# lichunshang/vision-enhanced-lidar-odometry

Hardware: AMD Instinct MI355X
Metric: scan-pairs/sec + achieved HBM GB/s, 120k-pt HDL-64E frame-to-frame ICP (higher is better)
Workload: dtype f32 association / f64 residuals+solve

## Files before the change

vision-enhanced-lidar-odometry_amd/csrc/velo_kernels.h:

```cpp
#pragma once
#include <hip/hip_runtime.h>
#include <stdint.h>

#include "velo_device_math.h"

#ifndef VELO_DEF_LOAD
#define VELO_DEF_LOAD 0
#endif
#ifndef VELO_DEF_ASSOC
#define VELO_DEF_ASSOC 0
#endif
#ifndef VELO_DEF_LMA
#define VELO_DEF_LMA 0
#endif
#ifndef VELO_DEF_LMB
#define VELO_DEF_LMB 0
#endif

namespace velo {

constexpr int kWave = 64;
constexpr int kNumAcc = 28;
constexpr int kEvalThreads = 256;
constexpr int kMaxEvalBlocks = 512;
// ... 490 lines not shown
    for (int off = 1; off < 64; off <<= 1) {
#pragma unroll
        for (int k = 0; k < kSub; k++) { const int t = __shfl_up(inc[k], off); if (lane >= off) inc[k] += t; }
    }
    if (lane == 63) {
#pragma unroll
        for (int k = 0; k < kSub; k++) s_wsum[k][wid] = inc[k];
    }
    __syncthreads();
    int ex[kSub], run = 0;
#pragma unroll
    for (int k = 0; k < kSub; k++) {
        int before = 0, all = 0;
#pragma unroll
        for (int w = 0; w < kWaves; w++) { const int sw = s_wsum[k][w]; if (w < wid) before += sw; all += sw; }
        ex[k] = run + before + inc[k] - ((v[k].x + v[k].y) + (v[k].z + v[k].w));
        run += all;
    }
    const int total = run;
    if (threadIdx.x == 0) {
        s_prefix = 0;
        __hip_atomic_store(&status[tile], (tile == 0 ? kLbPrefix : kLbAgg) | (unsigned long long)(unsigned)total, __ATOMIC_RELAXED, __HIP_MEMORY_SCOPE_AGENT);
    }
    if (tile > 0 && threadIdx.x < 64) {
        int acc = 0;
        for (int idx = tile - 1;; idx -= 64) {
            const int j = idx - lane;
            unsigned long long w = kLbPrefix;
            if (j >= 0) { do { w = __hip_atomic_load(&status[j], __ATOMIC_RELAXED, __HIP_MEMORY_SCOPE_AGENT); } while ((w & kLbFlags) == 0ull); }
            const unsigned long long pm = __ballot((w & kLbFlags) == kLbPrefix);
            const int first = (int)__ffsll((long long)pm) - 1;
            int val = (pm == 0ull || lane <= first) ? (int)(unsigned)(w & 0xffffffffull) : 0;
#pragma unroll
            for (int off = 32; off > 0; off >>= 1) val += __shfl_xor(val, off);
            acc += val;
            if (pm != 0ull) break;
        }
        if (lane == 0) {
            s_prefix = acc;
            __hip_atomic_store(&status[tile], kLbPrefix | (unsigned long long)(unsigned)(acc + total), __ATOMIC_RELAXED, __HIP_MEMORY_SCOPE_AGENT);
        }
    }
    __syncthreads();
    const int pre = s_prefix;
#pragma unroll
    for (int k = 0; k < kSub; k++) {
        const int i = tbase + k * (kScanThreads * 4) + threadIdx.x * 4;
        int4 q;
        q.x = pre + ex[k]; q.y = q.x + v[k].x; q.z = q.y + v[k].y; q.w = q.z + v[k].z;
        if (i + 3 < n) *reinterpret_cast<int4*>(data + i) = q;
        else { if (i < n) data[i] = q.x; if (i + 1 < n) data[i + 1] = q.y; if (i + 2 < n) data[i + 2] = q.z; }
        if (i <= n - 1 && n - 1 < i + 4) *grand_total = q.w + v[k].w;
    }
}
template <int kLbItems>
__global__ void __launch_bounds__(kScanThreads)
scan_lookback_kernel(int* __restrict__ data, int n, unsigned long long* __restrict__ status, int* __restrict__ ticket, int* __restrict__ grand_total) {
    scan_lookback_body<kLbItems>(data, n, status, ticket, grand_total);
}
__global__ void scan_tiles_kernel(int* __restrict__ data, int n, int* __restrict__ tile_sums)
#if VELO_DEF_LOAD
{
    const int base = blockIdx.x * kScanTile + threadIdx.x * kScanItems;
    int v[kScanItems], s = 0;
#pragma unroll
    for (int k = 0; k < kScanItems; k++) { v[k] = (base + k < n) ? data[base + k] : 0; s += v[k]; }
    int total;
    int ex = block_exclusive_scan(s, &total);
#pragma unroll
    for (int k = 0; k < kScanItems; k++) { if (base + k < n) data[base + k] = ex; ex += v[k]; }
    if (threadIdx.x == 0) tile_sums[blockIdx.x] = total;
}
#else
;
#endif
__global__ void scan_sums_kernel(int* __restrict__ tile_sums, int n_tiles, int* __restrict__ grand_total)
#if VELO_DEF_LOAD
{
    __shared__ int carry_s;
    if (threadIdx.x == 0) carry_s = 0;
    __syncthreads();
    for (int start = 0; start < n_tiles; start += kScanThreads) {
        const int i = start + threadIdx.x;
        const int v = (i < n_tiles) ? tile_sums[i] : 0;
        int total;
        const int ex = block_exclusive_scan(v, &total);
        const int carry = carry_s;
        if (i < n_tiles) tile_sums[i] = ex + carry;
        __syncthreads();
        if (threadIdx.x == 0) carry_s = carry + total;
        __syncthreads();
    }
    if (threadIdx.x == 0) *grand_total = carry_s;
}
#else
;
#endif
__global__ void scan_add_kernel(int* __restrict__ data, int n, const int* __restrict__ tile_sums, const int* __restrict__ grand_total,
                                int* __restrict__ cursor)
#if VELO_DEF_LOAD
{
    const int i = blockIdx.x * blockDim.x + threadIdx.x;
    if (i < n) { const int v = data[i] + tile_sums[i / kScanTile]; data[i] = v; cursor[i] = v; }
    else if (i == n) data[n] = *grand_total;
}
#else
;
#endif
__device__ __forceinline__ void grid_scatter_body(const float4* __restrict__ pts, const int* __restrict__ cell_of, const int* __restrict__ ring_of, int n,
                                                  int* __restrict__ cursor, const int* __restrict__ n_finite, int first_point,
                                                  float4* __restrict__ sorted, int* __restrict__ sring, const int bx) {
    const int i = bx * 256 + threadIdx.x;
    if (i < kGridPad) {
        const int j = *n_finite + i;
        sorted[j] = make_float4(__builtin_inff(), __builtin_inff(), __builtin_inff(), __int_as_float(0x7fffffff));
        sring[j] = 0x7fffffff;
    }
    const int c = i < n ? cell_of[i] : -1;
    bool head; int first, len;
    const int lane = threadIdx.x & 63;
    run_of_lane(c, lane, &head, &first, &len);
    int slot = head ? atomicAdd(&cursor[c], len) : 0;
    slot = __shfl(slot, first) + (lane - first);
    if (c < 0) return;
    const float4 p = pts[i];
    sorted[slot] = make_float4(p.x, p.y, p.z, __int_as_float(i + first_point));
    sring[slot] = ring_of[i];
}
__global__ void __launch_bounds__(256)
grid_scatter_kernel(const float4* __restrict__ pts, const int* __restrict__ cell_of, const int* __restrict__ ring_of, int n,
                    int* __restrict__ cursor, const int* __restrict__ n_finite, int first_point, float4* __restrict__ sorted, int* __restrict__ sring)
#if VELO_DEF_LOAD
{
    grid_scatter_body(pts, cell_of, ring_of, n, cursor, n_finite, first_point, sorted, sring, (int)blockIdx.x);
}
#else
;
#endif

constexpr int kAdvRings = 64, kAdvJobs = 4;
struct AdvJob {
    const float4* tgt; int* tgt_off_dev; int* ring_of; float4* pad; unsigned long long* lb_status; int* cell_of; int* table;
    float4* sorted; int* sring; int* scan_total; int* lb_ticket; int* clear; int n_clear;
    GridDesc g;
    int n_t, n_rings_t, first_ring, first_point, lb_words, nb_t, nc, n_tiles, nb_sc;
    const char* raw; long long stride; float4* src; int* src_off_dev; int* q_src; float4* qpts; unsigned* keys; unsigned* keys_next;
    unsigned* h_keys;
    float4* seed_fill;
    int n_s, n_rings_s, nb_pack, nb_q, skip, nq, patch, patch_rings, patch_len;
    int off_t[kAdvRings + 1], off_s[kAdvRings + 1];
};
struct AdvBatch { AdvJob job[kAdvJobs]; };

__global__ void __launch_bounds__(256)
advance_clear_kernel(AdvBatch B)
#if VELO_DEF_LOAD
{
    const AdvJob& J = B.job[blockIdx.y];
    int4* p = reinterpret_cast<int4*>(J.clear);
    const int n4 = J.n_clear >> 2;
    for (int i = blockIdx.x * 256 + threadIdx.x; i < n4; i += gridDim.x * 256) p[i] = make_int4(0, 0, 0, 0);
}
#else
;
#endif
__global__ void __launch_bounds__(256)
advance_ingest_kernel(AdvBatch B)
#if VELO_DEF_LOAD
{
    const AdvJob& J = B.job[blockIdx.y];
    __shared__ int s_off[kAdvRings + 2], s_qoff[kAdvRings + 2];
    __shared__ float red[4][6];
    const int tid = threadIdx.x, lane = tid & 63;
    int bx = blockIdx.x;
    if (bx < J.nb_t) {
        const int R = J.n_rings_t, n = J.n_t;
        if (tid <= R) s_off[tid] = J.off_t[tid];
        for (int j = bx * 256 + tid; j < J.lb_words; j += J.nb_t * 256) J.lb_status[j] = 0ull;
        __syncthreads();
        if (bx == 0 && tid <= R) J.tgt_off_dev[tid] = s_off[tid];
#pragma unroll
        for (int u = 0; u < kIngestPerThread; u++) {
            const int i = (bx * kIngestPerThread + u) * 256 + tid;
            int c = -1;
            if (i < n) {
                const float4 p = J.tgt[i];
                int lo = 0, hi = R;
                while (hi - lo > 1) { const int mid = (lo + hi) >> 1; if (s_off[mid] <= i) lo = mid; else hi = mid; }
                J.ring_of[i] = lo + J.first_ring;
                const int base = s_off[lo], end = s_off[lo + 1];
                J.pad[i + 2 * lo + 1] = p;
                if (i == base) J.pad[end + 2 * lo + 1] = p;
                if (i == end - 1) J.pad[base + 2 * lo] = p;
                if (isfinite(p.x) && isfinite(p.y) && isfinite(p.z)) c = cell_of_point(J.g, p);
                J.cell_of[i] = c;
            }
            bool head; int first, len;
            run_of_lane(c, lane, &head, &first, &len);
            if (head) atomicAdd(&J.table[c + 1], len);
        }
        return;
    }
    bx -= J.nb_t;
    if (bx >= J.nb_pack) return;
    const int R = J.n_rings_s;
    if (tid <= R) s_off[tid] = J.off_s[tid];
    if (tid < 64) {
        int cnt = tid < R ? (J.off_s[tid + 1] - J.off_s[tid] + J.skip - 1) / J.skip : 0;
#pragma unroll
        for (int o = 1; o < 64; o <<= 1) { const int t = __shfl_up(cnt, o); if (lane >= o) cnt += t; }
        if (tid == 0) s_qoff[0] = 0;
        if (tid < R) s_qoff[tid + 1] = cnt;
    }
    __syncthreads();
    if (bx == 0) {
        if (tid <= R) { J.src_off_dev[tid] = s_off[tid]; J.src_off_dev[R + 1 + tid] = s_qoff[tid]; }
        if (tid < 6) J.keys_next[tid] = tid < 3 ? 0xffffffffu : 0u;
    }
    if (bx >= J.nb_pack) return;
    __shared__ float s_raw[256 * 3];
    const int i = bx * 256 + tid;
    const bool have = i < J.n_s;
    const bool aligned = (reinterpret_cast<unsigned long long>(J.raw) & 15ull) == 0ull;
    float4 v = make_float4(0.f, 0.f, 0.f, 0.f);
    if (J.stride == 12 && aligned) {
        const char* base = J.raw + (long long)bx * 3072;
        const int nbytes = min(3072, (J.n_s - bx * 256) * 12);
        if (tid < 192) {
            if (tid * 16 + 16 <= nbytes) *reinterpret_cast<uint4*>(&s_raw[tid * 4]) = *reinterpret_cast<const uint4*>(base + tid * 16);
            else for (int f = 0; f < 4; f++) if (tid * 16 + 4 * f + 4 <= nbytes) s_raw[tid * 4 + f] = *reinterpret_cast<const float*>(base + tid * 16 + 4 * f);
        }
        __syncthreads();
        if (have) v = make_float4(s_raw[3 * tid], s_raw[3 * tid + 1], s_raw[3 * tid + 2], 0.0f);
    } else if (have) {
        const char* q = J.raw + (long long)i * J.stride;
        if (J.stride == 16 && aligned) { const float4 w = *reinterpret_cast<const float4*>(q); v = make_float4(w.x, w.y, w.z, 0.0f); }
        else { const float* p = reinterpret_cast<const float*>(q); v = make_float4(p[0], p[1], p[2], 0.0f); }
    }
    float mn[3] = {3.0e38f, 3.0e38f, 3.0e38f}, mx[3] = {-3.0e38f, -3.0e38f, -3.0e38f};
    if (have) {
        J.src[i] = v;
        if (isfinite(v.x) && isfinite(v.y) && isfinite(v.z)) { mn[0] = mx[0] = v.x; mn[1] = mx[1] = v.y; mn[2] = mx[2] = v.z; }
        if (J.nq > 0) {
            int lo = 0, hi = R;
            while (hi - lo > 1) { const int mid = (lo + hi) >> 1; if (s_off[mid] <= i) lo = mid; else hi = mid; }
            const int j = i - s_off[lo];
            if (j % J.skip == 0) {
                const int k = j / J.skip;
                const int pos = J.patch ? patch_position(s_qoff, R, lo, k, J.patch_rings, J.patch_len) : s_qoff[lo] + k;
                J.q_src[pos] = i;
                if (J.qpts) J.qpts[pos] = v;
                if (J.seed_fill) {
                    const float4 none = make_float4(__int_as_float(-1), __int_as_float(-1), __int_as_float(-1), __int_as_float(-1));
                    J.seed_fill[pos] = none; J.seed_fill[J.nq + pos] = none;
                }
            }
        }
    }
#pragma unroll
    for (int k = 0; k < 3; k++) {
#pragma unroll
        for (int o = 32; o > 0; o >>= 1) { mn[k] = fminf(mn[k], __shfl_xor(mn[k], o)); mx[k] = fmaxf(mx[k], __shfl_xor(mx[k], o)); }
    }
    const int wid = tid >> 6;
    if (lane == 0) { for (int k = 0; k < 3; k++) { red[wid][k] = mn[k]; red[wid][3 + k] = mx[k]; } }
    __syncthreads();
    if (tid < 6) {
        const int k = tid;
        float vv = red[0][k];
        for (int w = 1; w < 4; w++) vv = (k < 3) ? fminf(vv, red[w][k]) : fmaxf(vv, red[w][k]);
        const unsigned key = f2key(vv), cur = J.keys[k];
        if (k < 3) { if (vv < 3.0e38f && key < cur) atomicMin(&J.keys[k], key); } else { if (vv > -3.0e38f && key > cur) atomicMax(&J.keys[k], key); }
    }
}
#else
;
#endif
template <int kLbItems>
__global__ void __launch_bounds__(kScanThreads)
advance_scan_kernel(AdvBatch B) {
    const AdvJob& J = B.job[blockIdx.y];
    if ((int)blockIdx.x >= J.n_tiles) return;
    scan_lookback_body<kLbItems>(J.table + 1, J.nc, J.lb_status, J.lb_ticket, J.scan_total);
}
__global__ void __launch_bounds__(256)
advance_scatter_kernel(AdvBatch B)
#if VELO_DEF_LOAD
{
    const AdvJob& J = B.job[blockIdx.y];
    if ((int)blockIdx.x >= J.nb_sc) return;
    if (blockIdx.x == 0 && threadIdx.x < 6 && J.h_keys) J.h_keys[threadIdx.x] = J.keys[threadIdx.x];
    grid_scatter_body(J.tgt, J.cell_of, J.ring_of, J.n_t, J.table + 1, J.scan_total, J.first_point, J.sorted, J.sring, (int)blockIdx.x);
}
#else
;
#endif

struct PartialRec;
struct AssocOut {
    float4* __restrict__ p;
    float4* __restrict__ n;
    float4* __restrict__ v0;
    int4* __restrict__ aux0;
    float4* __restrict__ aux1;
    int* __restrict__ n_valid;
    int* __restrict__ n_valid_next;
    unsigned long long* __restrict__ dbg;
    unsigned long long* __restrict__ wg_times;
    int first_ring, first_point;
    struct PartialRec* __restrict__ partial;
    float4* __restrict__ prev_a;
    float4* __restrict__ prev_b;
    int2* __restrict__ prev_r;
    int* __restrict__ ask_count;
    int* __restrict__ ask_count_next;
    int* __restrict__ ask_list;
    unsigned long long* __restrict__ ask_keys;
    int2* __restrict__ ask_rings;
    int ask_map;
};

struct PartialRec {
    unsigned long long key1, key2;
    int ring1, ring2;
    int idx1, idx_k, idx2, pad;
    float v0[3], v2[3], v1[3];
    float pad2;
};

__device__ __forceinline__ float dist2_f(float qx, float qy, float qz, float sx, float sy, float sz) {
    const float dx = qx - sx, dy = qy - sy, dz = qz - sz;
    float r = dx * dx;
    r = r + dy * dy;
    r = r + dz * dz;
    return r;
}

__device__ __forceinline__ void transform_query(const PoseScalars& P, const float4& p, float* qx, float* qy, float* qz) {
    const double x = p.x, y = p.y, z = p.z;
    double r0, r1, r2;
    if (!P.small) {
        const double c0 = P.u[1] * z - P.u[2] * y, c1 = P.u[2] * x - P.u[0] * z, c2 = P.u[0] * y - P.u[1] * x;
        const double tmp = (P.u[0] * x + P.u[1] * y + P.u[2] * z) * P.omc;
        r0 = x * P.c + c0 * P.s + P.u[0] * tmp;
        r1 = y * P.c + c1 * P.s + P.u[1] * tmp;
        r2 = z * P.c + c2 * P.s + P.u[2] * tmp;
    } else {
        r0 = x + (P.w[1] * z - P.w[2] * y);
        r1 = y + (P.w[2] * x - P.w[0] * z);
        r2 = z + (P.w[0] * y - P.w[1] * x);
    }
    *qx = (float)(r0 + P.t[0]);
    *qy = (float)(r1 + P.t[1]);
    *qz = (float)(r2 + P.t[2]);
}

__device__ __forceinline__ int plane_from_points(const float v0[3], const float v1[3], const float v2[3], double norm_cond, float n[3]) {
    const float ax = v1[0] - v0[0], ay = v1[1] - v0[1], az = v1[2] - v0[2];
    const float bx = v2[0] - v0[0], by = v2[1] - v0[1], bz = v2[2] - v0[2];
    const float cx = ay * bz - az * by, cy = az * bx - ax * bz, cz = ax * by - ay * bx;
    const float nn = sqrtf(cx * cx + cy * cy + cz * cz);
    if ((double)nn < norm_cond) return 0;
    n[0] = cx / nn; n[1] = cy / nn; n[2] = cz / nn;
    return 1;
}

__device__ __forceinline__ void write_correspondence(int qi, const float4& psrc, int valid, const float n[3], const float v0[3],
                                                     int ring_i, int idx_i, int ring_j, int idx_j, int idx_k, float di, float dj,
                                                     const AssocOut& out, bool want_aux) {
    out.p[qi] = make_float4(psrc.x, psrc.y, psrc.z, __int_as_float(valid));
    out.n[qi] = valid ? make_float4(n[0], n[1], n[2], 0.f) : make_float4(0.f, 0.f, 0.f, 0.f);
    out.v0[qi] = valid ? make_float4(v0[0], v0[1], v0[2], 0.f) : make_float4(0.f, 0.f, 0.f, 0.f);
    if (want_aux) {
        out.aux0[qi] = make_int4(ring_i, idx_i, ring_j, idx_j);
        out.aux1[qi] = make_float4(__int_as_float(idx_k), di, dj, 0.f);
    }
    const unsigned long long m = __ballot(valid);
    const unsigned long long act = __ballot(1);
    if ((int)(threadIdx.x & 63) == (int)__ffsll((long long)act) - 1 && m) atomicAdd(out.n_valid, (int)__popcll(m));
}

__device__ __forceinline__ void finish_correspondence(
    int qi, const float4& psrc, float qx, float qy, float qz, unsigned long long b1, unsigned long long b2, unsigned long long key_inf,
    const float4* __restrict__ tgt, const int* __restrict__ tgt_off, const int* __restrict__ ring_of, double norm_cond,
    const AssocOut& out, bool want_aux) {
    int ring_i = -1, idx_i = 0, ring_j = -1, idx_j = 0, idx_k = 0;
    float di = 1e18f, dj = 1e18f;
    float v0[3] = {0.f, 0.f, 0.f}, v1[3] = {0.f, 0.f, 0.f}, v2[3] = {0.f, 0.f, 0.f};
    if (b1 < key_inf) {
        const int gi = (int)(unsigned)(b1 & 0xffffffffull) - out.first_point;
        ring_i = ring_of[gi];
        const int base = tgt_off[ring_i - out.first_ring];
        const int n = tgt_off[ring_i - out.first_ring + 1] - base;
        idx_i = gi - base;
        di = __uint_as_float((unsigned)(b1 >> 32));
        const int k1 = (idx_i + 1) % n, k2 = (idx_i - 1 + n) % n;
        const float4 a1 = tgt[base + k1], a2 = tgt[base + k2];
        const float d1 = dist2_f(a1.x, a1.y, a1.z, qx, qy, qz);
        const float d2 = dist2_f(a2.x, a2.y, a2.z, qx, qy, qz);
        idx_k = (d1 < d2) ? k1 : k2;
        const float4 p0 = tgt[base + idx_i];
        const float4 p2 = (idx_k == k1) ? a1 : a2;
        v0[0] = p0.x; v0[1] = p0.y; v0[2] = p0.z; v2[0] = p2.x; v2[1] = p2.y; v2[2] = p2.z;
    }
    if (b2 < key_inf) {
        const int gj = (int)(unsigned)(b2 & 0xffffffffull) - out.first_point;
        ring_j = ring_of[gj];
        idx_j = gj - tgt_off[ring_j - out.first_ring];
        dj = __uint_as_float((unsigned)(b2 >> 32));
        const float4 p1 = tgt[gj];
        v1[0] = p1.x; v1[1] = p1.y; v1[2] = p1.z;
    }
    if (out.partial) {
        PartialRec r;
        r.key1 = b1; r.key2 = b2; r.ring1 = ring_i; r.ring2 = ring_j; r.idx1 = idx_i; r.idx_k = idx_k; r.idx2 = idx_j; r.pad = 0;
        for (int k = 0; k < 3; k++) { r.v0[k] = v0[k]; r.v2[k] = v2[k]; r.v1[k] = v1[k]; }
        r.pad2 = 0.f;
        out.partial[qi] = r;
        return;
    }
    int valid = 0;
    float n[3] = {0.f, 0.f, 0.f};
    if (ring_i >= 0 && ring_j >= 0) valid = plane_from_points(v0, v1, v2, norm_cond, n);
    write_correspondence(qi, psrc, valid, n, v0, ring_i, idx_i, ring_j, idx_j, idx_k, di, dj, out, want_aux);
}

__device__ __forceinline__ void finish_correspondence_pad(
    int qi, const float4* __restrict__ qpts, float qx, float qy, float qz, unsigned long long b1, unsigned long long b2, int ring_i_in, int ring_j_in,
    unsigned long long key_inf, const float4* __restrict__ pad, const int* __restrict__ tgt_off, double norm_cond,
    const AssocOut& out, bool want_aux) {
    const bool has1 = b1 < key_inf, has2 = b2 < key_inf;
    const int gi = has1 ? (int)(unsigned)(b1 & 0xffffffffull) - out.first_point : 0;
    const int gj = has2 ? (int)(unsigned)(b2 & 0xffffffffull) - out.first_point : 0;
    const int li = has1 ? ring_i_in - out.first_ring : 0, lj = has2 ? ring_j_in - out.first_ring : 0;
    const int pi = gi + 2 * li + 1, pj = gj + 2 * lj + 1;
    const float4 psrc = qpts[qi];
    float4 p0 = make_float4(0.f, 0.f, 0.f, 0.f), p1 = p0, a1 = p0, a2 = p0;
    if (has1) { p0 = pad[pi]; a1 = pad[pi + 1]; a2 = pad[pi - 1]; }
    if (has2) p1 = pad[pj];
    int ring_i = -1, idx_i = 0, ring_j = -1, idx_j = 0, idx_k = 0;
    float di = 1e18f, dj = 1e18f;
    float v0[3] = {0.f, 0.f, 0.f}, v1[3] = {0.f, 0.f, 0.f}, v2[3] = {0.f, 0.f, 0.f};
    bool next_closer = false;
    if (has1) {
        ring_i = ring_i_in;
        di = __uint_as_float((unsigned)(b1 >> 32));
        const float d1 = dist2_f(a1.x, a1.y, a1.z, qx, qy, qz);
        const float d2 = dist2_f(a2.x, a2.y, a2.z, qx, qy, qz);
        next_closer = d1 < d2;
// ... 2781 lines not shown
    for (int i = 0; i < 6; i++) { sc[i] = S->scale[i]; gs[i] = S->g[i] * sc[i]; }
    const double scr = S->scale[r];
#pragma unroll
    for (int c = 0; c < 6; c++) {
        const double h = S->H[r <= c ? tri(r, c) : tri(c, r)];
        hrow[c] = h * scr * sc[c];
    }
    const int ei = lane < 36 ? lane / 6 : 5, ej = lane < 36 ? lane % 6 : 5;
    const double hs_e = S->H[ei <= ej ? tri(ei, ej) : tri(ej, ei)] * S->scale[ei] * S->scale[ej];
    int iter = S->iter, invalid = S->invalid, reuse = S->reuse_diag;
    double radius = S->radius, decrease = S->decrease;
    double diag_r = S->diag[r];
    for (;;) {
        if (iter + 1 > Q.max_num_iterations) { if (lane == 0) { S->done = 1; S->termination = 1; } break; }
        if (radius < Q.min_radius) { if (lane == 0) { S->done = 1; S->termination = 0; } break; }
        iter++;
        if (!reuse) {
            double hdd = hrow[0];
#pragma unroll
            for (int c = 1; c < 6; c++) hdd = (r == c) ? hrow[c] : hdd;
            diag_r = fmin(fmax(hdd, Q.min_diag), Q.max_diag);
        }
        const double inv_radius = 1.0 / radius;
        const double dterm = diag_r * inv_radius;
        double L[6], inv[6];
        bool ok = true;
#pragma unroll
        for (int j = 0; j < 6; j++) {
            double sj = (r == j) ? hrow[j] + dterm : hrow[j];
#pragma unroll
            for (int k = 0; k < j; k++) sj -= L[k] * lane_get(L[k], j);
            const double d = lane_get(sj, j);
            if (!(d > 0.0) || !isfinite(d)) { ok = false; break; }
            const double ljj = sqrt(d);
            inv[j] = 1.0 / ljj;
            L[j] = (r == j) ? ljj : sj * inv[j];
        }
        double y[6];
        if (ok) {
            double acc = gs[0];
#pragma unroll
            for (int c = 1; c < 6; c++) acc = (r == c) ? gs[c] : acc;
            double z[6];
#pragma unroll
            for (int k = 0; k < 6; k++) {
                z[k] = lane_get(acc, k) * inv[k];
                acc -= L[k] * z[k];
            }
#pragma unroll
            for (int i = 5; i >= 0; i--) {
                double sv = z[i];
#pragma unroll
                for (int k = i + 1; k < 6; k++) sv -= lane_get(L[i], k) * y[k];
                y[i] = sv * inv[i];
            }
#pragma unroll
            for (int i = 0; i < 6; i++) ok = ok && isfinite(y[i]);
        }
        reuse = 1;
        double mc = 0.0, step[6];
        if (ok) {
            double gd = 0.0, dHd = 0.0;
#pragma unroll
            for (int i = 0; i < 6; i++) step[i] = -y[i];
            double si = step[0], sj = step[0];
#pragma unroll
            for (int c = 1; c < 6; c++) { si = (ei == c) ? step[c] : si; sj = (ej == c) ? step[c] : sj; }
            const double prod = si * hs_e * sj;
#pragma unroll
            for (int i = 0; i < 6; i++) gd += gs[i] * step[i];
#pragma unroll
            for (int l = 0; l < 36; l++) dHd += lane_get(prod, l);
            mc = -(gd + 0.5 * dHd);
            if (!(mc > 0.0)) ok = false;
        }
        if (!ok) {
            if (++invalid >= Q.max_invalid) { if (lane == 0) { S->done = 1; S->termination = 2; } break; }
            radius = radius / decrease; decrease *= 2.0; reuse = 1;
            continue;
        }
        invalid = 0;
        if (lane == 0) {
            double dn = 0.0;
#pragma unroll
            for (int i = 0; i < 6; i++) { const double d = step[i] * sc[i]; S->xc[i] = S->x[i] + d; dn += d * d; }
            S->step_norm = sqrt(dn);
            S->model_change = mc;
            S->phase = PHASE_CAND;
        }
        break;
    }
    if (lane < 6) S->diag[lane] = diag_r;
    if (lane == 0) { S->iter = iter; S->invalid = invalid; S->reuse_diag = reuse; S->radius = radius; S->decrease = decrease; }
}
__device__ __forceinline__ void lm_transition_wave(const LMParams& Q, LMState* sL, const double* E, int lane) {
    int need = 0;
    if (lane == 0) {
        LMState L = *sL;
        bool ns = false;
        lm_transition_local(Q, &L, E, &ns);
        *sL = L;
        need = ns ? 1 : 0;
    }
    __builtin_amdgcn_fence(__ATOMIC_RELEASE, "wavefront");
    __builtin_amdgcn_wave_barrier();
    __builtin_amdgcn_fence(__ATOMIC_ACQUIRE, "wavefront");
    need = __builtin_amdgcn_readfirstlane(need);
    if (need) lm_compute_step_wave(Q, sL, lane);
    __builtin_amdgcn_fence(__ATOMIC_RELEASE, "wavefront");
    __builtin_amdgcn_wave_barrier();
    __builtin_amdgcn_fence(__ATOMIC_ACQUIRE, "wavefront");
}

__global__ void __launch_bounds__(256)
lm_step_kernel(LMParams Q, LMState* S, LMEvalPoint* pt, const double* __restrict__ partials, int n_blocks, unsigned long long* trace, int trace_eval,
               PoseRecord* __restrict__ pose_out, SolveLog* __restrict__ log)
#if VELO_DEF_LMA
{
    lm_transition(Q, S, pt, partials, n_blocks, trace, trace_eval, nullptr, pose_out, log);
}
#else
;
#endif
__global__ void __launch_bounds__(256)
lm_step_peer_kernel(LMParams Q, LMState* S, LMEvalPoint* pt, const double* __restrict__ partials, int n_blocks, PeerComm C,
                    PoseRecord* __restrict__ pose_out, SolveLog* __restrict__ log)
#if VELO_DEF_LMA
{
    lm_transition(Q, S, pt, partials, n_blocks, nullptr, 0, &C, pose_out, log);
}
#else
;
#endif
__global__ void lm_begin_batch_kernel(const LMBatchItem* __restrict__ items)
#if VELO_DEF_LMA
{
    const LMBatchItem& it = items[blockIdx.x];
    lm_begin_body(it.S, const_cast<LMEvalPoint*>(it.A.pt), it.xd, it.n_valid);
    if (threadIdx.x == 0 && it.pose_out) it.pose_out->ready = 0;
}
#else
;
#endif
__global__ void __launch_bounds__(256)
lm_step_batch_kernel(LMParams Q, const LMBatchItem* __restrict__ items)
#if VELO_DEF_LMA
{
    const LMBatchItem& it = items[blockIdx.x];
    lm_transition(Q, it.S, const_cast<LMEvalPoint*>(it.A.pt), it.A.partials, it.n_rows, nullptr, 0, nullptr, it.pose_out, it.log);
}
#else
;
#endif
template <bool M_LDS, int PRE, int CHUNK, bool VIS = false>
__device__ __forceinline__ void eval_step_batch_body(const LMParams& Q, const LMBatchItem& it, int* __restrict__ tickets, const int first) {
    const int bx = blockIdx.x, nbx = it.nb_icp, nb_all = VIS ? it.nb_icp + it.nb_vis : it.nb_icp;
    if (bx >= nb_all) return;
#ifdef VELO_LM_SETPRIO
    __builtin_amdgcn_s_setprio(VELO_LM_SETPRIO);
#endif
    const EvalArgs& A = it.A;
    const RowPrefetchT<PRE> f = prefetch_rows<PRE>(A, (VIS && bx >= nbx) ? 0 : bx, nbx);
    __shared__ LMEvalPoint s_pt;
    __shared__ LMState sL;
    __shared__ double s_scratch[CHUNK * kNumAcc];
    __shared__ int s_last;
    static_assert(CHUNK * kNumAcc >= kScratchDoubles / 2, "the sweep's reduction needs 64 columns x 28");
    if (first) {
        if (threadIdx.x < 4) {
            double x[6];
#pragma unroll
            for (int k = 0; k < 6; k++) x[k] = it.xd ? it.xd[k] : it.S->x[k];
            eval_point_column(x, 0, threadIdx.x, &s_pt);
        }
        __syncthreads();
    } else
    if (!eval_point_load(A, &s_pt)) return;
    double acc[kNumAcc];
    if (VIS && bx >= nbx) {
        if (M_LDS) visual_sweep_one(A, s_pt, bx - nbx, it.nb_vis, acc);
        else visual_sweep_acc(A, s_pt, bx - nbx, it.nb_vis, acc);
        block_reduce_store<true>(acc, A.partials + (size_t)(A.vis_row0 + bx - nbx) * kNumAcc, s_scratch);
    } else {
        sweep_rows<M_LDS, PRE>(A, f, s_pt, bx, nbx, acc);
        block_reduce_store<true>(acc, A.partials + (size_t)bx * kNumAcc, s_scratch);
    }
    asm volatile("s_waitcnt vmcnt(0)" ::: "memory");
    __syncthreads();
    if (threadIdx.x == 0) s_last = __hip_atomic_fetch_add(tickets + blockIdx.y, 1, __ATOMIC_RELAXED, __HIP_MEMORY_SCOPE_AGENT) == nb_all - 1 ? 1 : 0;
    __syncthreads();
    if (!s_last) return;
    if (threadIdx.x == 0) __hip_atomic_store(tickets + blockIdx.y, 0, __ATOMIC_RELAXED, __HIP_MEMORY_SCOPE_AGENT);
    lm_advance<true, CHUNK, false, true>(Q, it.S, A.partials, it.n_rows, first ? 2 : 0, it.xd, it.n_valid, s_scratch, &sL, &s_pt, nullptr, 0, nullptr, it.pose_out, it.log);
    const int t = threadIdx.x;
    LMEvalPoint* pt = const_cast<LMEvalPoint*>(A.pt);
    if (t < (int)(sizeof(LMState) / 8)) reinterpret_cast<unsigned long long*>(it.S)[t] = reinterpret_cast<const unsigned long long*>(&sL)[t];
    else if (t >= 64 && t < 64 + (int)(sizeof(LMEvalPoint) / 8)) reinterpret_cast<unsigned long long*>(pt)[t - 64] = reinterpret_cast<const unsigned long long*>(&s_pt)[t - 64];
}
__global__ void __launch_bounds__(kEvalThreads)
eval_step_batch_kernel(LMParams Q, const LMBatchItem* __restrict__ items, int* __restrict__ tickets, int first)
#if VELO_DEF_LMB
{
    eval_step_batch_body<false, kPre, kStepChunk>(Q, items[blockIdx.y], tickets, first);
}
#else
;
#endif
#ifndef VELO_LEAN_PRE
#define VELO_LEAN_PRE 1
#endif
__global__ void __launch_bounds__(kEvalThreads) __attribute__((amdgpu_num_vgpr(152)))
eval_step_batch_lean_kernel(LMParams Q, const LMBatchItem* __restrict__ items, int* __restrict__ tickets, int first)
#if VELO_DEF_LMB
{
    eval_step_batch_body<true, VELO_LEAN_PRE, 64>(Q, items[blockIdx.y], tickets, first);
}
#else
;
#endif
__global__ void __launch_bounds__(kEvalThreads) __attribute__((amdgpu_num_vgpr(152)))
eval_step_batch_lean_vis_kernel(LMParams Q, const LMBatchItem* __restrict__ items, int* __restrict__ tickets, int first)
#if VELO_DEF_LMB
{
    eval_step_batch_body<true, VELO_LEAN_PRE, 64, true>(Q, items[blockIdx.y], tickets, first);
}
#else
;
#endif
__global__ void __launch_bounds__(kEvalThreads)
eval_step_batch_vis_kernel(LMParams Q, const LMBatchItem* __restrict__ items, int* __restrict__ tickets, int first)
#if VELO_DEF_LMB
{
    eval_step_batch_body<false, kPre, kStepChunk, true>(Q, items[blockIdx.y], tickets, first);
}
#else
;
#endif
struct LMBatchPackV { LMBatchItem item[4]; };
__global__ void __launch_bounds__(kEvalThreads)
eval_step_batch_v_kernel(LMParams Q, LMBatchPackV P, int* __restrict__ tickets, int first)
#if VELO_DEF_LMB
{
    eval_step_batch_body<false, kPre, kStepChunk>(Q, P.item[blockIdx.y], tickets, first);
}
#else
;
#endif
__global__ void __launch_bounds__(kEvalThreads) __attribute__((amdgpu_num_vgpr(152)))
eval_step_batch_lean_v_kernel(LMParams Q, LMBatchPackV P, int* __restrict__ tickets, int first)
#if VELO_DEF_LMB
{
    eval_step_batch_body<true, VELO_LEAN_PRE, 64>(Q, P.item[blockIdx.y], tickets, first);
}
#else
;
#endif
__global__ void __launch_bounds__(kEvalThreads) __attribute__((amdgpu_num_vgpr(152)))
eval_step_batch_lean_vis_v_kernel(LMParams Q, LMBatchPackV P, int* __restrict__ tickets, int first)
#if VELO_DEF_LMB
{
    eval_step_batch_body<true, VELO_LEAN_PRE, 64, true>(Q, P.item[blockIdx.y], tickets, first);
}
#else
;
#endif
template <bool M_LDS, int PRE, int CHUNK>
__device__ __forceinline__ void lm_iter_lean_body(const EvalArgs& A, const LMParams& Q, const LMState* __restrict__ Sin, LMState* __restrict__ Sout,
                                                  const double* __restrict__ pin, int n_in, double* __restrict__ pout, int first,
                                                  const double* __restrict__ x_in, const int* __restrict__ n_valid, const int bx, const int nbx,
                                                  PoseRecord* pose_out, SolveLog* log) {
    __shared__ LMState sL;
    __shared__ LMEvalPoint s_pt;
    __shared__ double s_scratch[CHUNK * kNumAcc];
    const RowPrefetchT<PRE> f = prefetch_rows<PRE>(A, bx, nbx);
    lm_advance<false, CHUNK>(Q, Sin, pin, n_in, first, x_in, n_valid, s_scratch, &sL, &s_pt, nullptr, 0, nullptr, pose_out, log, bx == 0);
    const int t = threadIdx.x;
    if (bx == 0 && t < (int)(sizeof(LMState) / 8)) reinterpret_cast<unsigned long long*>(Sout)[t] = reinterpret_cast<const unsigned long long*>(&sL)[t];
    if (sL.done) return;
    double acc[kNumAcc];
    sweep_rows<M_LDS, PRE>(A, f, s_pt, bx, nbx, acc);
    block_reduce_store(acc, pout + (size_t)bx * kNumAcc, s_scratch);
}
__global__ void __launch_bounds__(kEvalThreads) __attribute__((amdgpu_num_vgpr(152)))
lm_iter_batch_lean_kernel(LMParams Q, LMBatchPackV P, int parity, int first, size_t half)
#if VELO_DEF_LMB
{
    const LMBatchItem& it = P.item[blockIdx.y];
    if ((int)blockIdx.x >= it.nb_icp) return;
    lm_iter_lean_body<true, VELO_LEAN_PRE, 64>(it.A, Q, it.S + parity, it.S + (parity ^ 1), it.A.partials + (size_t)parity * half, it.nb_icp,
                                               it.A.partials + (size_t)(parity ^ 1) * half, first, it.xd, it.n_valid, blockIdx.x, it.nb_icp, it.pose_out, it.log);
}
#else
;
#endif
__device__ __forceinline__ int ctl_load(const int* p) { return __hip_atomic_load(p, __ATOMIC_RELAXED, __HIP_MEMORY_SCOPE_AGENT); }
__device__ __forceinline__ void ctl_store(int* p, int v) { __hip_atomic_store(p, v, __ATOMIC_RELAXED, __HIP_MEMORY_SCOPE_AGENT); }
#ifndef VELO_TEST_ATTR
#define VELO_TEST_ATTR __attribute__((amdgpu_num_vgpr(152)))
#endif
struct AgCtl { int epoch, abort, pad[30]; int flag[2][kMaxEvalBlocks]; };

struct SolveCtl { int ticket, pad0[31]; int arrived, pad1[31]; int gen, pad2[31]; int exited, pad3[31]; };
constexpr int kSolveDone = 1 << 30;
template <int PRE>
__device__ __forceinline__ int persist_sweep(const EvalArgs& A, SolveCtl* __restrict__ ctl, const int k, const int bx, const int nb,
                                             LMEvalPoint* s_pt, double* s_scratch, int* s_flag) {
    const int t = threadIdx.x;
    const LMEvalPoint* pt = A.pt;
    const RowPrefetchT<PRE> f = prefetch_rows<PRE>(A, bx, nb);
    if (t == 0) {
        int fl = 0;
        for (;;) {
            const int g = ctl_load(&ctl->gen);
            if (g & kSolveDone) { fl = 1; break; }
            if (g > k) break;
            __builtin_amdgcn_s_sleep(8);
        }
        *s_flag = fl;
    }
    __syncthreads();
    const int over = *s_flag;
    __syncthreads();
    if (over) return -1;
    if (t < (int)(sizeof(LMEvalPoint) / 8))
        reinterpret_cast<unsigned long long*>(s_pt)[t] = __hip_atomic_load(reinterpret_cast<const unsigned long long*>(pt) + t, __ATOMIC_RELAXED, __HIP_MEMORY_SCOPE_AGENT);
    __syncthreads();
    double acc[kNumAcc];
#ifndef VELO_T2
    sweep_rows<true, PRE>(A, f, *s_pt, bx, nb, acc);
#else
    for (int q = 0; q < kNumAcc; q++) acc[q] = f.p[0].x;
#endif
    block_reduce_store<true>(acc, A.partials + (size_t)bx * kNumAcc, s_scratch);
    asm volatile("s_waitcnt vmcnt(0)" ::: "memory");
    __syncthreads();
    if (t == 0) *s_flag = __hip_atomic_fetch_add(&ctl->arrived, 1, __ATOMIC_RELAXED, __HIP_MEMORY_SCOPE_AGENT) == nb - 1 ? 1 : 0;
    __syncthreads();
    const int last = *s_flag;
    __syncthreads();
    return last;
}
__device__ __attribute__((noinline)) void persist_advance(const LMParams* Q, const LMBatchItem* it, int first, double* s_scratch, LMState* sL, LMEvalPoint* s_pt) {
    lm_advance<true, 64, true>(*Q, it->S, it->A.partials, it->n_rows, first, it->xd, it->n_valid, s_scratch, sL, s_pt, nullptr, 0, nullptr, it->pose_out, it->log);
}
template <int PRE>
__device__ __forceinline__ void lm_solve_persist_body(const LMParams& Q, const LMBatchItem* __restrict__ item, SolveCtl* __restrict__ ctl, const int kmax, const int n_wgs) {
    __shared__ LMEvalPoint s_pt;
    __shared__ LMState sL;
    __shared__ double s_scratch[64 * kNumAcc];
    __shared__ int s_ticket, s_flag;
    const int t = threadIdx.x;
    bool running = true;
    while (running) {
        const LMBatchItem* itp = item;
        asm volatile("" : "+s"(itp));
        const LMBatchItem& it = *itp;
        const EvalArgs& A = it.A;
        const int nb = it.nb_icp;
        LMEvalPoint* pt = const_cast<LMEvalPoint*>(A.pt);
        if (t == 0) s_ticket = __hip_atomic_fetch_add(&ctl->ticket, 1, __ATOMIC_RELAXED, __HIP_MEMORY_SCOPE_AGENT);
        __syncthreads();
        const int tk = s_ticket;
        __syncthreads();
        const int k = (tk - 1) / nb, bx = (tk - 1) - k * nb;
        int advance = 0;
        if (tk == 0) advance = 1;
        else if (k >= kmax) running = false;
        else {
            const int r = persist_sweep<PRE>(A, ctl, k, bx, nb, &s_pt, s_scratch, &s_flag);
            if (r < 0) running = false;
            else if (r > 0) advance = 2;
        }
        if (advance) {
            if (advance == 2 && t == 0) ctl_store(&ctl->arrived, 0);
#ifndef VELO_T1
            persist_advance(&Q, itp, advance == 1 ? 1 : 0, s_scratch, &sL, &s_pt);
#endif
            if (t < (int)(sizeof(LMState) / 8)) __hip_atomic_store(reinterpret_cast<unsigned long long*>(it.S) + t, reinterpret_cast<const unsigned long long*>(&sL)[t], __ATOMIC_RELAXED, __HIP_MEMORY_SCOPE_AGENT);
            else if (t >= 64 && t < 64 + (int)(sizeof(LMEvalPoint) / 8)) __hip_atomic_store(reinterpret_cast<unsigned long long*>(pt) + (t - 64), reinterpret_cast<const unsigned long long*>(&s_pt)[t - 64], __ATOMIC_RELAXED, __HIP_MEMORY_SCOPE_AGENT);
            asm volatile("s_waitcnt vmcnt(0)" ::: "memory");
            __syncthreads();
            if (t == 0) ctl_store(&ctl->gen, (advance == 1 ? 1 : k + 2) | (sL.done ? kSolveDone : 0));
            __syncthreads();
        }
    }
    __syncthreads();
    if (t == 0 && __hip_atomic_fetch_add(&ctl->exited, 1, __ATOMIC_RELAXED, __HIP_MEMORY_SCOPE_AGENT) == n_wgs - 1) {
        ctl_store(&ctl->ticket, 0); ctl_store(&ctl->arrived, 0); ctl_store(&ctl->gen, 0); ctl_store(&ctl->exited, 0);
    }
}
__global__ void __launch_bounds__(kEvalThreads, 3)
lm_solve_persist_batch_kernel(LMParams Q, const LMBatchItem* __restrict__ items, SolveCtl* __restrict__ ctl, int kmax)
#if VELO_DEF_LMB
{
    lm_solve_persist_body<VELO_LEAN_PRE>(Q, items + blockIdx.y, ctl + blockIdx.y, kmax, (int)gridDim.x);
}
#else
;
#endif

__global__ void lm_gather_states_kernel(const LMBatchItem* __restrict__ items, LMState* __restrict__ out, int which)
#if VELO_DEF_LMB
{
    const unsigned* src = reinterpret_cast<const unsigned*>(items[blockIdx.x].S + which);
    unsigned* dst = reinterpret_cast<unsigned*>(out + blockIdx.x);
    for (int k = threadIdx.x; k < (int)(sizeof(LMState) / 4); k += blockDim.x) dst[k] = src[k];
}
#else
;
#endif

constexpr int kFinishJobs = 8;
struct ChainFinish {
    const LMState* S[kFinishJobs];
// ... 246 lines not shown
```

Baseline: 4204.

## Let next-frame advance phases ride as extra workgroups on LM step kernels

Splits the advance clear/ingest/scan/scatter kernels into device bodies and adds a rider path in the lean LM step kernels. Workgroups past a launch offset encoded in `ride` run one advance phase for the next frame, with the step's scratch LDS reused for ingest. The aim is to overlap next-frame grid construction with LM iterations and save separate kernel launches. The risks are higher LDS use per step workgroup and a kernel signature change that needs host launch updates. That host update is not visible here, so the change may be inactive if `ride` is passed as 0.

```diff
diff --git a/vision-enhanced-lidar-odometry_amd/csrc/velo_kernels.h b/vision-enhanced-lidar-odometry_amd/csrc/velo_kernels.h
--- a/vision-enhanced-lidar-odometry_amd/csrc/velo_kernels.h
+++ b/vision-enhanced-lidar-odometry_amd/csrc/velo_kernels.h
@@ -666,27 +666,25 @@
 };
 struct AdvBatch { AdvJob job[kAdvJobs]; };
 
+__device__ __forceinline__ void advance_clear_body(const AdvJob& J, const int bx, const int nbx) {
+    int4* p = reinterpret_cast<int4*>(J.clear);
+    const int n4 = J.n_clear >> 2;
+    for (int i = bx * 256 + threadIdx.x; i < n4; i += nbx * 256) p[i] = make_int4(0, 0, 0, 0);
+}
 __global__ void __launch_bounds__(256)
 advance_clear_kernel(AdvBatch B)
 #if VELO_DEF_LOAD
 {
-    const AdvJob& J = B.job[blockIdx.y];
-    int4* p = reinterpret_cast<int4*>(J.clear);
-    const int n4 = J.n_clear >> 2;
-    for (int i = blockIdx.x * 256 + threadIdx.x; i < n4; i += gridDim.x * 256) p[i] = make_int4(0, 0, 0, 0);
-}
-#else
-;
-#endif
-__global__ void __launch_bounds__(256)
-advance_ingest_kernel(AdvBatch B)
-#if VELO_DEF_LOAD
-{
-    const AdvJob& J = B.job[blockIdx.y];
-    __shared__ int s_off[kAdvRings + 2], s_qoff[kAdvRings + 2];
-    __shared__ float red[4][6];
+    advance_clear_body(B.job[blockIdx.y], (int)blockIdx.x, (int)gridDim.x);
+}
+#else
+;
+#endif
+struct alignas(16) AdvIngestLds { int s_off[kAdvRings + 2], s_qoff[kAdvRings + 2]; float red[4][6]; float s_raw[256 * 3]; };
+__device__ __forceinline__ void advance_ingest_body(const AdvJob& J, int bx, AdvIngestLds& L) {
+    int* const s_off = L.s_off; int* const s_qoff = L.s_qoff;
+    float (* const red)[6] = L.red; float* const s_raw = L.s_raw;
     const int tid = threadIdx.x, lane = tid & 63;
-    int bx = blockIdx.x;
     if (bx < J.nb_t) {
         const int R = J.n_rings_t, n = J.n_t;
         if (tid <= R) s_off[tid] = J.off_t[tid];
@@ -732,7 +730,6 @@
         if (tid < 6) J.keys_next[tid] = tid < 3 ? 0xffffffffu : 0u;
     }
     if (bx >= J.nb_pack) return;
-    __shared__ float s_raw[256 * 3];
     const int i = bx * 256 + tid;
     const bool have = i < J.n_s;
     const bool aligned = (reinterpret_cast<unsigned long long>(J.raw) & 15ull) == 0ull;
@@ -787,28 +784,47 @@
         if (k < 3) { if (vv < 3.0e38f && key < cur) atomicMin(&J.keys[k], key); } else { if (vv > -3.0e38f && key > cur) atomicMax(&J.keys[k], key); }
     }
 }
-#else
-;
-#endif
+__global__ void __launch_bounds__(256)
+advance_ingest_kernel(AdvBatch B)
+#if VELO_DEF_LOAD
+{
+    __shared__ AdvIngestLds L;
+    advance_ingest_body(B.job[blockIdx.y], (int)blockIdx.x, L);
+}
+#else
+;
+#endif
+template <int kLbItems>
+__device__ __forceinline__ void advance_scan_body(const AdvJob& J, const int bx) {
+    if (bx >= J.n_tiles) return;
+    scan_lookback_body<kLbItems>(J.table + 1, J.nc, J.lb_status, J.lb_ticket, J.scan_total);
+}
 template <int kLbItems>
 __global__ void __launch_bounds__(kScanThreads)
 advance_scan_kernel(AdvBatch B) {
-    const AdvJob& J = B.job[blockIdx.y];
-    if ((int)blockIdx.x >= J.n_tiles) return;
-    scan_lookback_body<kLbItems>(J.table + 1, J.nc, J.lb_status, J.lb_ticket, J.scan_total);
+    advance_scan_body<kLbItems>(B.job[blockIdx.y], (int)blockIdx.x);
+}
+__device__ __forceinline__ void advance_scatter_body(const AdvJob& J, const int bx) {
+    if (bx >= J.nb_sc) return;
+    if (bx == 0 && threadIdx.x < 6 && J.h_keys) J.h_keys[threadIdx.x] = J.keys[threadIdx.x];
+    grid_scatter_body(J.tgt, J.cell_of, J.ring_of, J.n_t, J.table + 1, J.scan_total, J.first_point, J.sorted, J.sring, bx);
 }
 __global__ void __launch_bounds__(256)
 advance_scatter_kernel(AdvBatch B)
 #if VELO_DEF_LOAD
 {
-    const AdvJob& J = B.job[blockIdx.y];
-    if ((int)blockIdx.x >= J.nb_sc) return;
-    if (blockIdx.x == 0 && threadIdx.x < 6 && J.h_keys) J.h_keys[threadIdx.x] = J.keys[threadIdx.x];
-    grid_scatter_body(J.tgt, J.cell_of, J.ring_of, J.n_t, J.table + 1, J.scan_total, J.first_point, J.sorted, J.sring, (int)blockIdx.x);
-}
-#else
-;
-#endif
+    advance_scatter_body(B.job[blockIdx.y], (int)blockIdx.x);
+}
+#else
+;
+#endif
+constexpr int kAdvRidePhases = 4;
+__device__ __forceinline__ void advance_rider(const AdvJob& J, const int phase, const int bx, const int nbx, void* lds) {
+    if (phase == 1) advance_clear_body(J, bx, nbx);
+    else if (phase == 2) advance_ingest_body(J, bx, *reinterpret_cast<AdvIngestLds*>(lds));
+    else if (phase == 3) advance_scan_body<kLbItemsSmall>(J, bx);
+    else if (phase == 4) advance_scatter_body(J, bx);
+}
 
 struct PartialRec;
 struct AssocOut {
@@ -3896,8 +3912,20 @@
 #else
 ;
 #endif
-template <bool M_LDS, int PRE, int CHUNK, bool VIS = false>
-__device__ __forceinline__ void eval_step_batch_body(const LMParams& Q, const LMBatchItem& it, int* __restrict__ tickets, const int first) {
+#ifdef VELO_UNIT_LM_ONLY
+struct AdvBatch;
+#endif
+template <bool M_LDS, int PRE, int CHUNK, bool VIS = false, bool RIDE = false>
+__device__ __forceinline__ void eval_step_batch_body(const LMParams& Q, const LMBatchItem& it, int* __restrict__ tickets, const int first,
+                                                     const AdvBatch* __restrict__ adv = nullptr, const int ride = 0) {
+    __shared__ __attribute__((aligned(16))) double s_scratch[CHUNK * kNumAcc];
+#ifndef VELO_UNIT_LM_ONLY
+    if (RIDE && ride != 0 && (int)blockIdx.x >= (ride >> 3)) {
+        static_assert(!RIDE || sizeof(AdvIngestLds) <= sizeof(double) * CHUNK * kNumAcc, "a carried ingest workgroup's LDS comes out of the step's scratch");
+        advance_rider(adv->job[blockIdx.y], ride & 7, (int)blockIdx.x - (ride >> 3), (int)gridDim.x - (ride >> 3), s_scratch);
+        return;
+    }
+#endif
     const int bx = blockIdx.x, nbx = it.nb_icp, nb_all = VIS ? it.nb_icp + it.nb_vis : it.nb_icp;
     if (bx >= nb_all) return;
 #ifdef VELO_LM_SETPRIO
@@ -3907,7 +3935,6 @@
     const RowPrefetchT<PRE> f = prefetch_rows<PRE>(A, (VIS && bx >= nbx) ? 0 : bx, nbx);
     __shared__ LMEvalPoint s_pt;
     __shared__ LMState sL;
-    __shared__ double s_scratch[CHUNK * kNumAcc];
     __shared__ int s_last;
     static_assert(CHUNK * kNumAcc >= kScratchDoubles / 2, "the sweep's reduction needs 64 columns x 28");
     if (first) {
@@ -3991,19 +4018,19 @@
 ;
 #endif
 __global__ void __launch_bounds__(kEvalThreads) __attribute__((amdgpu_num_vgpr(152)))
-eval_step_batch_lean_v_kernel(LMParams Q, LMBatchPackV P, int* __restrict__ tickets, int first)
+eval_step_batch_lean_v_kernel(LMParams Q, LMBatchPackV P, int* __restrict__ tickets, int first, const AdvBatch* __restrict__ adv, int ride)
 #if VELO_DEF_LMB
 {
-    eval_step_batch_body<true, VELO_LEAN_PRE, 64>(Q, P.item[blockIdx.y], tickets, first);
+    eval_step_batch_body<true, VELO_LEAN_PRE, 64, false, true>(Q, P.item[blockIdx.y], tickets, first, adv, ride);
 }
 #else
 ;
 #endif
 __global__ void __launch_bounds__(kEvalThreads) __attribute__((amdgpu_num_vgpr(152)))
-eval_step_batch_lean_vis_v_kernel(LMParams Q, LMBatchPackV P, int* __restrict__ tickets, int first)
+eval_step_batch_lean_vis_v_kernel(LMParams Q, LMBatchPackV P, int* __restrict__ tickets, int first, const AdvBatch* __restrict__ adv, int ride)
 #if VELO_DEF_LMB
 {
-    eval_step_batch_body<true, VELO_LEAN_PRE, 64, true>(Q, P.item[blockIdx.y], tickets, first);
+    eval_step_batch_body<true, VELO_LEAN_PRE, 64, true, true>(Q, P.item[blockIdx.y], tickets, first, adv, ride);
 }
 #else
 ;
```

Result: slower. 4128 (-1.8%).
